# Yogesh352/llmsys-project-flashattn

Measured on AMD Instinct MI355X. Metric: FlashAttn fwd TFLOP/s (+ HBM GB/s) at (B,H,N,d)=(8,16,4096,64); 1/2/4/8 GPU, higher is better.
Workload: dtype bf16; 1 GPU; flash_attention_fwd c3; B=8, H=16, N=4096, d=64, causal=False, output=fp32 O, parallelism=bh-shard x1 (strong)

## Files before the change

### include/minitorch_hip.h

```cpp
#ifndef MINITORCH_HIP_H
#define MINITORCH_HIP_H

#include <stdint.h>
#include <stdbool.h>

#ifdef __cplusplus
extern "C" {
#endif

enum { MT_F32 = 0, MT_BF16 = 1, MT_BF16_F32OUT = 2 };

const char* mt_last_error(void);
int mt_abi_version(void);
int mt_flash_set_kernel_policy(int policy);
int mt_flash_get_kernel_policy(void);
int64_t mt_scratch_bytes(void);
int mt_scratch_release(void);

int mt_flash_attn_fwd(int dtype, int causal, const void* q, const void* k, const void* v,
                      void* o, float* m, float* l, int64_t B, int64_t H, int64_t N, int64_t d,
                      const int64_t* q_strides, const int64_t* k_strides,
                      const int64_t* v_strides, const int64_t* o_strides, void* stream);

int mt_flash_attn_fwd_varlen(int dtype, int causal, const void* q, const void* k, const void* v,
                             void* o, float* m, float* l, int64_t B, int64_t H, int64_t N,
                             int64_t d, const int64_t* q_strides, const int64_t* k_strides,
                             const int64_t* v_strides, const int64_t* o_strides,
                             const int* kv_len, void* stream);

int64_t mt_flash_attn_bwd_workspace_bytes(int64_t B, int64_t H, int64_t N, int64_t d);

int mt_flash_attn_bwd(int dtype, int causal, const void* q, const void* k, const void* v,
                      const void* o, const void* dout, const float* m, const float* l,
                      void* dq, void* dk, void* dv, int64_t B, int64_t H, int64_t N,
                      int64_t d, const int64_t* strides, void* workspace, void* stream);
int mt_flash_attn_bwd_varlen(int dtype, int causal, const void* q, const void* k, const void* v,
                             const void* o, const void* dout, const float* m, const float* l,
                             void* dq, void* dk, void* dv, int64_t B, int64_t H, int64_t N,
                             int64_t d, const int64_t* strides, const int* kv_len,
                             void* workspace, void* stream);
int mt_flash_attn_bwd_v3(int dtype, int causal, const void* q, const void* k, const void* v,
                         const void* o, const void* dout, const float* m, const float* l,
                         void* dq, void* dk, void* dv, int64_t B, int64_t H, int64_t N,
                         int64_t d, const int64_t* strides, const int* kv_len,
                         void* workspace, int64_t workspace_bytes, void* stream);

int mt_flash_attn_decode_splits(int dtype, int64_t B, int64_t H, int64_t Nq, int64_t Nk, int64_t d,
                                int64_t* span_keys, int64_t* tile_keys);
int64_t mt_flash_attn_decode_workspace_bytes(int dtype, int64_t B, int64_t H, int64_t Nq, int64_t Nk,
                                             int64_t d);
int mt_flash_attn_decode(int dtype, int causal, const void* q, const void* k_cache, const void* v_cache,
                         void* o, float* m, float* l, int64_t B, int64_t H, int64_t Nq, int64_t Nk,
                         int64_t d, const int64_t* q_strides, const int64_t* k_strides,
                         const int64_t* v_strides, const int64_t* o_strides, const int* kv_len,
                         void* workspace, int64_t workspace_bytes, void* stream);
int mt_flash_attn_decode_gqa_splits(int dtype, int64_t B, int64_t H, int64_t Hkv, int64_t Nq, int64_t Nk,
                                    int64_t d, int64_t* span_keys, int64_t* tile_keys);
int64_t mt_flash_attn_decode_gqa_workspace_bytes(int dtype, int64_t B, int64_t H, int64_t Hkv, int64_t Nq,
                                                 int64_t Nk, int64_t d);
int mt_flash_attn_decode_gqa(int dtype, int causal, const void* q, const void* k_cache, const void* v_cache,
                             void* o, float* m, float* l, int64_t B, int64_t H, int64_t Hkv, int64_t Nq,
                             int64_t Nk, int64_t d, const int64_t* q_strides, const int64_t* k_strides,
                             const int64_t* v_strides, const int64_t* o_strides, const int* kv_len,
                             void* workspace, int64_t workspace_bytes, void* stream);
int mt_flash_attn_extend_plan(int dtype, int64_t B, int64_t H, int64_t Hkv, int64_t Nq, int64_t Nk,
                              int64_t d, int64_t* block_queries, int64_t* tile_keys);
int mt_flash_attn_extend(int dtype, int causal, const void* q, const void* k_cache, const void* v_cache,
                         void* o, float* m, float* l, int64_t B, int64_t H, int64_t Hkv, int64_t Nq,
                         int64_t Nk, int64_t d, const int64_t* q_strides, const int64_t* k_strides,
                         const int64_t* v_strides, const int64_t* o_strides,
                         const int* kv_len, const int* q_len, void* stream);
int mt_kv_cache_append(int dtype, const void* k_new, const void* v_new, void* k_cache, void* v_cache,
                       int64_t B, int64_t H, int64_t Nq, int64_t Nmax, int64_t d,
                       const int64_t* knew_strides, const int64_t* vnew_strides,
                       const int64_t* kcache_strides, const int64_t* vcache_strides,
// ... 104 lines not shown
```

### llmsys-project-flashattn_amd/csrc/capi_flash.hip

```cpp
#include <stdarg.h>
#include <stdio.h>
#include <stdlib.h>
#include <string.h>

#include "../../include/minitorch_hip.h"
#include "fa_common.h"
#include <algorithm>
#include <atomic>
#include <mutex>
#include <vector>

namespace mt {
hipError_t launch_fwd_generic(const AttnArgs& a, bool bf16_io, bool vec, bool causal,
                              hipStream_t st, int ring);
hipError_t launch_fwd_fast(const AttnArgs& a, bool causal, int variant, hipStream_t st,
                           bool* handled);
hipError_t launch_fwd_v4(const AttnArgs& a, bool causal, int nw, bool pk, hipStream_t st,
                         bool* handled, int pair = 0);
hipError_t launch_fwd_v5(const AttnArgs& a, bool causal, int ahead, int var, hipStream_t st,
                         bool* handled);
hipError_t launch_fwd_v6(const AttnArgs& a, bool causal, int var, hipStream_t st, bool* handled);
hipError_t launch_fwd_d128(const AttnArgs& a, bool causal, int nw, bool dma, hipStream_t st,
                           bool* handled, int pair = 0);
hipError_t launch_fwd_d128v2(const AttnArgs& a, bool causal, int var, hipStream_t st, bool* handled);
hipError_t launch_bwd_bf16(const AttnArgs& a, bool causal, int variant, hipStream_t st, bool* handled);
hipError_t launch_bwd_generic(const AttnArgs& a, bool bf16_io, bool vec, bool causal,
                              hipStream_t st, int pair, bool ring, int64_t fused_slab);
int64_t bwd_fused_ws_bytes(int64_t B, int64_t H, int64_t N);
int64_t ring_fused_ws_bytes(int64_t B, int64_t H, int64_t N);
int64_t bwd_fused_abi2_bytes(int64_t B, int64_t H, int64_t N);
#ifdef MT_DIAGNOSTICS
hipError_t launch_fwd_v4_deep(const AttnArgs& a, bool causal, bool pk, hipStream_t st);
hipError_t launch_fwd_v4_ablation(const AttnArgs& a, int abl, hipStream_t st);
#endif

static thread_local char g_err[512] = "";

enum : int {
  kPolDefault = 0,
  kPolGeneric = 1,
  kPolFast8 = 2, kPolFast4 = 3, kPolFastSp8 = 4, kPolFastSp4 = 5, kPolFastPp = 6,
  kPolV4w4 = 21, kPolV4w8 = 22, kPolV4Pk8 = 23, kPolV4Pk4 = 24, kPolV4DeepPk = 25,
  kPolV4Deep = 26,
  kPolV4Pair4 = 50, kPolV4Pair8 = 51, kPolD128Pair4 = 52, kPolD128Pair8 = 53,
  kPolV4PairLF4 = 63, kPolV4PairLF8 = 64, kPolD128PairLF8 = 65,
  kPolV5a2 = 27, kPolV5a4 = 28, kPolV5a6 = 29, kPolV5NoUnroll = 31, kPolV5Dma = 35,
  kPolV5w8 = 36, kPolV5w8Dma = 37, kPolV5w4Reg = 38, kPolV5Prio = 39, kPolV5Scalar = 46,
  kPolV5Stagger = 47, kPolV5ScalarStagger = 48, kPolV5StaggerPrio = 49, kPolV5VKeep = 54,
  kPolV5VKeepPrio = 55, kPolV5Defer = 56, kPolV5Defer3 = 57, kPolV5Defer4 = 58,
  kPolV5AsmDma = 61,
  kPolV5Causal8 = 67, kPolV5Causal4 = 68,
  kPolD128w8 = 32, kPolD128w4 = 33, kPolD128Dma8 = 44, kPolD128Dma4 = 45,
  kPolBwdPipe = 40, kPolBwdQ32 = 43, kPolBwdQ64OneWave = 62,
  kPolBwdQ64Dma = 66, kPolBwdQ64Dma8 = 69,
  kPolBwdStagger = 70,
  kPolBwdDqPf = 71,
  kPolBwdMix0 = 74,
  kPolBwdMix4 = 75,
  kPolV5Split = 76,
  kPolBwdQ128 = 77,
  kPolV5RowSum = 78, kPolV5RowSumNoKeep = 79,
  kPolV6 = 100, kPolV6RowSum = 102, kPolV6RowSumNoKeep = 103,
  kPolV6RowSumEven = 104,
  kPolV6Split = 105,
  kPolV6Causal = 106,
  kPolBwdPair = 107, kPolBwdPair8 = 108,
  kPolFwdF32TwoBarrier = 109, kPolFwdF32Ring = 110, kPolFwdF32RingPair = 111,
  kPolBwdGenNoPair = 112, kPolBwdGenPair = 113,
  kPolBwdF32Lds = 114,
  kPolBwdFused = 120,
  kPolBwdSplit = 121,
  kPolD128v2 = 130, kPolD128v2Vs = 131, kPolD128v2Prio = 132, kPolD128v2w4 = 133, kPolD128v2w4Vs = 134,
  kPolD128v2Ah3 = 135, kPolD128v2Ah4 = 136,
  kPolD128v2Causal = 137,
// ... 266 lines not shown
    if (pol >= 80 && pol <= 86) {
      static const int kAbl[7] = {12, 28, 4, 68, 132, 260, 6};
      var = kAbl[pol - 80];
    }
    if (pol == 97) var = 2;
    if (pol == 98) var = v5::kDefault | 1048576;
    if (pol >= 91 && pol <= 96 && a.d == 64) {
      *handled = true;
      return launch_fwd_v4_ablation(a, pol - 90, st);
    }
#endif
    if (var >= 0) e = launch_fwd_v5(a, false, ahead, var, st, handled);
  }
  if (!*handled && pol == kPolDefault && causal && a.d == 64 &&
      (int64_t)((a.N + 511) / 512 + 1) / 2 * a.B * a.H >= 256)
  {
    const bool w4 = !a.o_f32 && (int64_t)((a.N + 255) / 256 + 1) / 2 * a.B * a.H >= 512;
    e = launch_fwd_v6(a, true, a.o_f32 ? 610 : w4 ? (98 | 16384) : 98, st, handled);
    if (!*handled) e = launch_fwd_v5(a, true, 2, v5::kDefault, st, handled);
  }
  if (!*handled && pol == kPolDefault && a.d == 64)
    e = launch_fwd_v4(a, causal, causal && N >= 8192 ? 8 : 4, !causal, st, handled,
                      causal ? 2 : 0);
  if (!*handled && a.d == 128) {
    int nw = -1, pair = 0;
    bool dma = false;
    if (pol == kPolDefault) e = launch_fwd_d128v2(a, causal, causal ? 32 : 0, st, handled);
    switch (*handled ? -1 : pol) {
      case kPolDefault: nw = 8; pair = causal ? 2 : 0; break;
      case kPolD128w8: nw = 8; break;
      case kPolD128w4: nw = 4; break;
      case kPolD128Dma8: nw = 8; dma = true; break;
      case kPolD128Dma4: nw = 4; dma = true; break;
      case kPolD128Pair4: nw = 4; pair = 1; break;
      case kPolD128Pair8: nw = 8; pair = 1; break;
      case kPolV4PairLF4: nw = 4; pair = 2; break;
      case kPolV4PairLF8: case kPolD128PairLF8: nw = 8; pair = 2; break;
      default: break;
    }
    if (nw > 0) e = launch_fwd_d128(a, causal, nw, dma, st, handled, pair);
  }
  if (!*handled) {
    int var = 2;
    if (pol >= kPolFast8 && pol <= kPolFastPp) var = pol;
#ifdef MT_DIAGNOSTICS
    if (pol >= 10 && pol <= 15) var = pol;
#endif
    e = launch_fwd_fast(a, causal, var, st, handled);
  }
  return e;
}
#endif

static hipError_t fwd_bf16_dispatch(const AttnArgs& a, bool causal, int pol, hipStream_t st,
                                    bool* handled) {
#ifdef MT_DIAGNOSTICS
  if (pol != kPolDefault && pol != kPolBwdFused && pol != kPolBwdSplit)
    return fwd_bf16_dispatch_ab(a, causal, pol, st, handled);
#endif
  (void)pol;
  *handled = false;
  hipError_t e = hipSuccess;
  const int N = a.N;
  const int64_t bh = (int64_t)a.B * a.H;
  if (a.d == 64) {
    if (!causal) {
      if (N % 64 == 0 && (int64_t)((N + 255) / 256) * bh >= 512)
        e = launch_fwd_v6(a, false, 66 | 16384, st, handled);
      else if ((int64_t)((N + 511) / 512) * bh >= 256)
        e = launch_fwd_v6(a, false, N % 64 ? 66 | 65536 : 66, st, handled);
      if (!*handled) e = launch_fwd_v6(a, false, 18, st, handled);
    } else {
      const int64_t w4grid = (int64_t)((N + 255) / 256 + 1) / 2 * bh;
      const int64_t w8grid = (int64_t)((N + 511) / 512 + 1) / 2 * bh;
      const int rg = N % 64 ? 65536 : 0;
      if (!a.o_f32 && w4grid >= 256) e = launch_fwd_v6(a, true, (98 | 16384) | rg, st, handled);
      else if (a.o_f32 && !rg && w8grid >= 256) e = launch_fwd_v6(a, true, 610, st, handled);
    }
    if (!*handled)
      e = launch_fwd_v4(a, causal, causal && N >= 8192 ? 8 : 4, !causal, st, handled, causal ? 2 : 0);
  }
  if (!*handled && a.d == 128) e = launch_fwd_d128v2(a, causal, causal ? 32 : 0, st, handled);
  if (!*handled && a.d == 128) e = launch_fwd_d128(a, causal, 8, false, st, handled, causal ? 2 : 0);
  if (!*handled) e = launch_fwd_fast(a, causal, 2, st, handled);
  return e;
}

}

using namespace mt;

extern "C" {

const char* mt_last_error(void) { return g_err; }
int mt_flash_set_kernel_policy(int policy) {
  if (!policy_valid(policy))
    return set_error("mt_flash_set_kernel_policy: unknown policy %d", policy);
  g_kernel_policy.store(policy, std::memory_order_relaxed);
  return 0;
}
int mt_flash_get_kernel_policy(void) { return g_kernel_policy.load(std::memory_order_relaxed); }
int mt_abi_version(void) { return 3; }

int mt_flash_attn_fwd(int dtype, int causal, const void* q, const void* k, const void* v,
                      void* o, float* m, float* l, int64_t B, int64_t H, int64_t N, int64_t d,
                      const int64_t* q_strides, const int64_t* k_strides,
                      const int64_t* v_strides, const int64_t* o_strides, void* stream) {
  return mt_flash_attn_fwd_varlen(dtype, causal, q, k, v, o, m, l, B, H, N, d, q_strides,
                                  k_strides, v_strides, o_strides, nullptr, stream);
}

int mt_flash_attn_fwd_varlen(int dtype, int causal, const void* q, const void* k, const void* v,
                             void* o, float* m, float* l, int64_t B, int64_t H, int64_t N,
                             int64_t d, const int64_t* q_strides, const int64_t* k_strides,
                             const int64_t* v_strides, const int64_t* o_strides,
                             const int* kv_len, void* stream) {
  const bool f32o = dtype == MT_BF16_F32OUT;
  if (f32o) dtype = MT_BF16;
  if (check_sizes(dtype, B, H, N, d)) return 1;
  if (!q || !k || !v || !o) return set_error("mt_flash_attn_fwd: null tensor pointer");
  AttnArgs a;
  memset(&a, 0, sizeof(a));
  a.q = q; a.k = k; a.v = v; a.out = o; a.m = m; a.l = l;
  a.kv_len = kv_len;
  a.o_f32 = f32o ? 1 : 0;
#ifdef MT_DIAGNOSTICS
  if (const char* kn = getenv("MT_KNOB")) a.knob = atoi(kn);
#endif
  fill_strides(a.sq, q_strides, H, N, d);
  fill_strides(a.sk, k_strides, H, N, d);
  fill_strides(a.sv, v_strides, H, N, d);
  fill_strides(a.so, o_strides, H, N, d);
  a.B = (int)B; a.H = (int)H; a.N = (int)N; a.d = (int)d;
  a.scale = (float)(1.0 / sqrt((double)d));
  a.scale_log2 = (float)(1.4426950408889634 / sqrt((double)d));
  const int es = dtype == MT_BF16 ? 2 : 4;
  const bool vec = vec_ok(d, es, {a.sq, a.sk, a.sv, a.so}, {q, k, v, o});
  if (f32o && !vec_ok(d, 4, {a.so}, {o}))
    return set_error("mt_flash_attn_fwd: an fp32 O needs 16-B aligned rows (d and O strides multiples of 4)");
  hipStream_t st = (hipStream_t)stream;
  const int pol = g_kernel_policy.load(std::memory_order_relaxed);
  if (dtype == MT_BF16 && vec && pol != kPolGeneric && !kv_len) {
    const int64_t dp = pad_dim(d);
    if (dp) {
      const int64_t oes = f32o ? 4 : 2;
      bool declined = false;
      const hipError_t e = for_head_groups(B, H, N * dp * (3 * 2 + oes), [&](int64_t b0, int64_t h0, int64_t nb, int64_t nh) -> hipError_t {
        if (declined) return hipSuccess;
        const int64_t nel = nb * nh * N * dp;
        char* buf = (char*)pad_scratch((size_t)(nel * (3 * 2 + oes)), st);
        if (!buf) { declined = true; return hipSuccess; }
        AttnArgs ap = a;
        ap.B = (int)nb; ap.H = (int)nh;
        ap.q = buf; ap.k = buf + nel * 2; ap.v = buf + nel * 4; ap.out = buf + nel * 6;
        int64_t* ps[4] = {ap.sq, ap.sk, ap.sv, ap.so};
// ... 303 lines not shown
```

### llmsys-project-flashattn_amd/csrc/fa_fwd_v6.hip

```cpp
#include "fa_fwd_bf16.h"

#ifndef V6ABL
#define V6ABL 0
#endif
#ifndef V6NT
#define V6NT 1
#endif

namespace mt {

namespace {

using namespace fwdbf16;
constexpr int D = 64;
constexpr int kBK = 64;
constexpr int TILE = kBK * D;
constexpr int kKSlots = 4, kVSlots = 2;
constexpr int kNW = 8;
constexpr int kBQ = 64 * kNW;
constexpr float kLimit = 1.8446744e19f;
constexpr float kThr = 8.0f;

typedef __attribute__((address_space(3))) s16x4 lds_s16x4;
typedef __attribute__((ext_vector_type(8))) short s16x8;
typedef __attribute__((ext_vector_type(4))) float f32x4;
typedef __attribute__((ext_vector_type(2))) float f32x2;
typedef __attribute__((ext_vector_type(8))) _Float16 f16x8;
typedef __attribute__((ext_vector_type(2))) _Float16 f16x2;
typedef __attribute__((ext_vector_type(4))) unsigned u32x4;

struct Blk6 {
  f32x4 s[4][2];
};
struct Pf6 {
  bf16x8 p[2];
};

__device__ __forceinline__ f32x4 mma16(const bf16x8& a, const bf16x8& b, const f32x4& c) {
  return __builtin_amdgcn_mfma_f32_16x16x32_bf16(a, b, c, 0, 0, 0);
}
template <bool H>
__device__ __forceinline__ f32x4 mma_pv(const bf16x8& a, const bf16x8& b, const f32x4& c) {
  if (!H) return mma16(a, b, c);
  return __builtin_amdgcn_mfma_f32_16x16x32_f16(__builtin_bit_cast(f16x8, a), __builtin_bit_cast(f16x8, b), c, 0, 0, 0);
}

__device__ __forceinline__ u32x4 vcvt_read(const bf16* tile, int tid) {
  return *(const u32x4*)((const char*)tile + tid * 16);
}
__device__ __forceinline__ void vcvt_write(bf16* tile, int tid, const u32x4& x) {
  u32x4 y;
#pragma unroll
  for (int j = 0; j < 4; ++j) {
    const f32x2 f = {__uint_as_float(x[j] << 16), __uint_as_float(x[j] & 0xffff0000u)};
    y[j] = __builtin_bit_cast(unsigned, __builtin_convertvector(f, f16x2));
  }
  *(u32x4*)((char*)tile + tid * 16) = y;
}

// ... 59 lines not shown

template <bool SOFT, bool PS, bool RS = false, bool EV = false, bool H = false, bool PK = false>
__device__ __forceinline__ void qk6(const bf16* sk, const int (&ko)[2], const bf16x8 (&qf)[2][2], Blk6& S,
                                    const f32x4 (&ci)[2], const Blk6& s_in, int kk, float c2,
                                    const float (&nmc)[2], f32x2 (&acc)[2], Pf6& pf) {
  bf16x8 kf[8];
  kf[0] = kread6(sk, ko, 0);
  kf[1] = kread6(sk, ko, 1);
  f32x2 ep, ec;
#pragma unroll
  for (int m = 0; m < 16; ++m) {
    const int f = m >> 1, kb = f >> 1, ks = f & 1, qh = m & 1;
    if (!(m & 1) && f + 2 < 8) kf[f + 2] = ((V6ABL & 1) && SOFT && f + 2 >= 4) ? kf[(f - 2) ^ 1] : kread6(sk, ko, f + 2);
    S.s[kb][qh] = mma16(kf[f], qf[qh][ks], ks ? S.s[kb][qh] : ci[qh]);
    if (SOFT) sm6_slot<PS, RS, EV, H, PK>(m, s_in, kk, c2, nmc, acc, pf, ep, ec);
    __builtin_amdgcn_sched_barrier(0);
  }
  if (SOFT && EV) sm6_fin<true, H>(ep, 7, acc, pf);
}

template <bool SOFT, int KEEP, bool PS, bool RS = false, bool EV = false, bool H = false, bool PK = false>
__device__ __forceinline__ void pv6(const bf16* sv, const int (&vo)[4], f32x4 (&O)[4][2], const Pf6& plo,
                                    const Pf6& phi, const Blk6& s_in, int kk, float c2,
                                    const float (&nmc)[2], f32x2 (&acc)[2], Pf6& pf, bf16x8 (&vk)[8],
                                    f32x4 (&R)[2]) {
  constexpr short one = H ? 0x3c00 : 0x3f80;
  const bf16x8 ones = __builtin_bit_cast(bf16x8, s16x8{one, one, one, one, one, one, one, one});
  bf16x8 vf_own[8];
  bf16x8(&vf)[8] = KEEP ? vk : vf_own;
  if (KEEP != 2) {
    vf[0] = vread6(sv, vo, 0);
    vf[1] = vread6(sv, vo, 1);
  }
  f32x2 ep, ec;
#pragma unroll
  for (int m = 0; m < 16; ++m) {
    const int f = m >> 1, hv = f >> 2, db = f & 3, qh = m & 1;
    if (KEEP != 2 && !(m & 1) && f + 2 < 8) vf[f + 2] = ((V6ABL & 8) && SOFT && f + 2 >= 4) ? vf[f - 2] : vread6(sv, vo, f + 2);
    O[db][qh] = mma_pv<H>(vf[f], (hv ? phi : plo).p[qh], O[db][qh]);
    if (RS && db == 0 && !((V6ABL & 2) && SOFT)) R[qh] = mma_pv<H>(ones, (hv ? phi : plo).p[qh], R[qh]);
    if (SOFT) sm6_slot<PS, RS, EV, H, PK>(m, s_in, kk, c2, nmc, acc, pf, ep, ec);
    __builtin_amdgcn_sched_barrier(0);
  }
  if (SOFT && EV) sm6_fin<true, H>(ep, 7, acc, pf);
}

__device__ __forceinline__ float quad_max(float x) {
  x = fmaxf(x, __shfl_xor(x, 16));
  return fmaxf(x, __shfl_xor(x, 32));
}
__device__ __forceinline__ float quad_sum(float x) {
  x += __shfl_xor(x, 16);
  return x + __shfl_xor(x, 32);
}
__device__ __forceinline__ float lane_max6(const Blk6& s, int qh) {
  float m = fmaxf(fmaxf(s.s[0][qh][0], s.s[0][qh][1]), s.s[0][qh][2]);
#pragma unroll
  for (int kb = 0; kb < 4; ++kb)
#pragma unroll
    for (int r = (kb ? 0 : 3); r < 4; ++r) m = fmaxf(m, s.s[kb][qh][r]);
  return m;
}

__device__ __forceinline__ void dma6(uint32_t lds, __amdgpu_buffer_rsrc_t rs, int go, int step) {
  unsigned keep;
  asm volatile(
      "s_mov_b32 %0, m0\n\ts_mov_b32 m0, %2\n\ts_nop 0\n\t"
      "buffer_load_dwordx4 %1, %3, 0 offen lds\n\ts_mov_b32 m0, %0"
      : "=&s"(keep)
      : "v"(go + step), "s"(lds), "s"(rs)
      : "memory");
}

__device__ __forceinline__ void dma6s(uint32_t lds, __amdgpu_buffer_rsrc_t rs, int go, int soff) {
  unsigned keep;
  asm volatile(
      "s_mov_b32 %0, m0\n\ts_mov_b32 m0, %2\n\ts_nop 0\n\t"
      "buffer_load_dwordx4 %1, %3, %4 offen lds\n\ts_mov_b32 m0, %0"
      : "=&s"(keep)
      : "v"(go), "s"(lds), "s"(rs), "s"(soff)
      : "memory");
}

}

template <int VAR>
__global__ __launch_bounds__(64 * kNW, 1) void fa_fwd_bf16_v6(AttnArgs p, int nqb) {
  constexpr bool PS = VAR & 1, RS = VAR & 2, EV = RS && (VAR & 8), SPLIT = VAR & 16, CAUSAL = VAR & 32;
  constexpr bool WIDE = VAR & 64;
  constexpr bool NOBAR = VAR & 128;
  constexpr bool DUAL = VAR & 256;
  constexpr bool H = VAR & 512;
  constexpr bool STAMP = VAR & 1024;
  constexpr bool ODMA = (VAR & 2048) && !SPLIT && !DUAL;
  constexpr int PFLIP = (VAR & 4096) ? 3 : (VAR & 8192) ? 2 : 0;
  constexpr bool W4 = (VAR & 16384) && !SPLIT && !DUAL;
  constexpr bool PK = (VAR & 32768) && !PS;
  constexpr bool RG = VAR & 65536;
  static_assert(!RG || (!SPLIT && !DUAL && !PS && (CAUSAL || !W4)), "ragged N: the 8-wave non-causal and the causal forms");
  constexpr bool RGM = RG && !CAUSAL;
  constexpr int NCV = W4 ? 2 : 1;
  static_assert(!(SPLIT && CAUSAL), "split keys: non-causal");
  static_assert(!DUAL || CAUSAL, "dual halves: causal");
  static_assert(!H || (CAUSAL && !DUAL && !PS && RS && !EV), "fp16 PV: the causal default form");
  constexpr int VS = H ? 4 : kVSlots;
  constexpr int K1 = (VAR & 4) ? 0 : 1, K2 = (VAR & 4) ? 0 : 2;
  constexpr int NWQ = (SPLIT || DUAL || W4) ? 4 : kNW;
  constexpr int LPT = ODMA ? 2 : kNW / NWQ;
  constexpr int BQ = 64 * NWQ;
  extern __shared__ __attribute__((aligned(16))) char smem_raw[];

  const int tid = threadIdx.x, lane = tid & 63;
  const int wave = __builtin_amdgcn_readfirstlane(tid >> 6);
  const int g = lane >> 4, i16 = lane & 15;
  const int N = p.N;
  const int half = (SPLIT || DUAL) ? (wave >> 2) : 0;
  const int wq = (SPLIT || DUAL) ? (wave & 3) : wave;
  const int Nk = SPLIT ? N / 2 : N;
  bf16* const sK = (bf16*)smem_raw + half * (kKSlots + VS) * TILE;
  bf16* const sV = sK + kKSlots * TILE;

  const int nblk = gridDim.x, hw = blockIdx.x;
  const int xcd = hw & 7, slot = hw >> 3, qd = nblk >> 3, rm = nblk & 7;
  const int logical = (xcd < rm ? xcd * (qd + 1) : rm * (qd + 1) + (xcd - rm) * qd) + slot;
  const int nunit = DUAL ? nqb / 4 : CAUSAL ? (nqb + 1) / 2 : nqb;
  const int bh = logical / nunit, qb = logical % nunit;
  const int b = bh / p.H, hh = bh % p.H;

  const bf16* Qg = (const bf16*)p.q + b * p.sq[0] + hh * p.sq[1];
  const bf16* Kg = (const bf16*)p.k + b * p.sk[0] + hh * p.sk[1] + (int64_t)(SPLIT ? half : 0) * Nk * p.sk[2];
  const bf16* Vg = (const bf16*)p.v + b * p.sv[0] + hh * p.sv[1] + (int64_t)(SPLIT ? half : 0) * Nk * p.sv[2];
  const int skn = (int)p.sk[2], svn = (int)p.sv[2];
  const __amdgpu_buffer_rsrc_t rk =
      __builtin_amdgcn_make_buffer_rsrc((void*)Kg, (short)0, ((Nk - 1) * skn + D) * 2, 0x00020000);
  const __amdgpu_buffer_rsrc_t rv =
      __builtin_amdgcn_make_buffer_rsrc((void*)Vg, (short)0, ((Nk - 1) * svn + D) * 2, 0x00020000);

  int ko[2], vo[4];
#pragma unroll
  for (int ks = 0; ks < 2; ++ks) ko[ks] = k_swz<D>(i16, 4 * ks + g);
  {
    const int q = i16 >> 2, pp = i16 & 3, row = 4 * g + q;
#pragma unroll
    for (int db = 0; db < 4; ++db)
      vo[db] = row * D + (((2 * db + (pp >> 1)) ^ (((row >> 1) & 3) << 1)) * 8) + 4 * (pp & 1);
  }
  auto prow = [&](int i) __attribute__((always_inline)) { return W4 ? 8 * (wq + 4 * i) : 8 * (LPT * wq + i); };
  constexpr int NDO = W4 ? 1 : LPT;
  int kdo[NDO], vdo[NDO];
#pragma unroll
  for (int i = 0; i < NDO; ++i) {
    const int dr = prow(i) + (lane >> 3), dc = lane & 7;
    kdo[i] = (dr * skn + (dc ^ ((dr >> 1) & 7)) * 8) * 2;
// ... 278 lines not shown
        const int qf0 = qw + 32 * blk;
        if (CAUSAL && (qf0 + 31 < t * kBK || qf0 >= N)) continue;
        Blk6 S;
        f32x2 acc[2] = {f32x2{0.f, 0.f}, f32x2{0.f, 0.f}};
        Pf6 plo, phi, dpf;
        const float z[2] = {0.f, 0.f};
        qk6<false, false>(sK, ko, blk ? qfB : qfA, S, ci0, S, 0, c2, z, acc, dpf);
        if (RGM && t * kBK + kBK > Nk) {
#pragma unroll
          for (int kb = 0; kb < 4; ++kb)
#pragma unroll
            for (int qh = 0; qh < 2; ++qh)
#pragma unroll
              for (int r = 0; r < 4; ++r)
                if (t * kBK + 16 * kb + 4 * g + r >= Nk) S.s[kb][qh][r] = -INFINITY;
        }
        if (CAUSAL && t * kBK + kBK - 1 > qf0) {
#pragma unroll
          for (int kb = 0; kb < 4; ++kb)
#pragma unroll
            for (int qh = 0; qh < 2; ++qh)
#pragma unroll
              for (int r = 0; r < 4; ++r)
                if (t * kBK + 16 * kb + 4 * g + r > qf0 + 16 * qh + i16) S.s[kb][qh][r] = -INFINITY;
        }
        float(&m)[2] = blk ? mB : mA;
        float(&l)[2] = blk ? pB : pA;
        f32x4(&O)[4][2] = blk ? OB : OA;
        float nmc[2];
#pragma unroll
        for (int qh = 0; qh < 2; ++qh) {
          const float tmax = quad_max(lane_max6(S, qh));
          if (__builtin_amdgcn_ballot_w64((tmax - m[qh]) * c2e > kThr)) {
            const float m_new = fmaxf(m[qh], tmax);
            const float alpha = m[qh] == -INFINITY ? 0.f : __builtin_amdgcn_exp2f((m[qh] - m_new) * c2e);
            m[qh] = m_new;
#pragma unroll
            for (int db = 0; db < 4; ++db) O[db][qh] *= alpha;
            l[qh] *= alpha;
          }
          nmc[qh] = -(m[qh] * c2e);
        }
#pragma unroll
        for (int i = 0; i < 8; ++i) sm6_fin(sm6_exp<false>(S, 0, i, c2e, nmc), i, acc, plo);
#pragma unroll
        for (int i = 0; i < 8; ++i) sm6_fin(sm6_exp<false>(S, 1, i, c2e, nmc), i, acc, phi);
#pragma unroll
        for (int qh = 0; qh < 2; ++qh) l[qh] += acc[qh][0] + acc[qh][1];
        f32x2 d2[2];
        f32x4 dR[2];
        pv6<false, 0, false>(sV, vo, O, plo, phi, S, 0, c2, nmc, d2, dpf, vk, dR);
      }
    }
  }
  if (SPLIT) {
    __syncthreads();
    float4* xch = (float4*)smem_raw + wq * 18 * 64 + lane;
    if (half) {
#pragma unroll
      for (int db = 0; db < 4; ++db)
#pragma unroll
        for (int qh = 0; qh < 2; ++qh) {
          const f32x4 a = OA[db][qh], o = OB[db][qh];
          xch[(2 * db + qh) * 64] = make_float4(a[0], a[1], a[2], a[3]);
          xch[(8 + 2 * db + qh) * 64] = make_float4(o[0], o[1], o[2], o[3]);
        }
      xch[16 * 64] = make_float4(mA[0], mA[1], mB[0], mB[1]);
      xch[17 * 64] = make_float4(pA[0], pA[1], pB[0], pB[1]);
    }
    __syncthreads();
    if (half) return false;
    const float4 tm = xch[16 * 64], tp = xch[17 * 64];
    const float om[4] = {tm.x, tm.y, tm.z, tm.w}, op[4] = {tp.x, tp.y, tp.z, tp.w};
#pragma unroll
    for (int blk = 0; blk < 2; ++blk)
#pragma unroll
      for (int qh = 0; qh < 2; ++qh) {
        float& m = blk ? mB[qh] : mA[qh];
        float& l = blk ? pB[qh] : pA[qh];
        const float n = fmaxf(m, om[2 * blk + qh]);
        const float a0 = __builtin_amdgcn_exp2f((m - n) * c2e), a1 = __builtin_amdgcn_exp2f((om[2 * blk + qh] - n) * c2e);
#pragma unroll
        for (int db = 0; db < 4; ++db) {
          const float4 u = xch[((blk ? 8 : 0) + 2 * db + qh) * 64];
          f32x4& o = (blk ? OB : OA)[db][qh];
          o = o * a0 + f32x4{u.x, u.y, u.z, u.w} * a1;
        }
        l = l * a0 + op[2 * blk + qh] * a1;
        m = n;
      }
  }

#pragma unroll
  for (int blk = 0; blk < 2; ++blk) {
#pragma unroll
    for (int qh = 0; qh < 2; ++qh) {
      const int q = qw + 32 * blk + 16 * qh + i16;
      const float l = quad_sum(blk ? pB[qh] : pA[qh]);
      const float m = blk ? mB[qh] : mA[qh];
      const float inv = 1.f / l;
      const f32x4(&O)[4][2] = blk ? OB : OA;
      if (V6ABL & 16) {
        float t = 0.f;
#pragma unroll
        for (int db = 0; db < 4; ++db) t += O[db][qh][0] * inv + O[db][qh][1] + O[db][qh][2] + O[db][qh][3];
        if (t == 1.2345e-30f) p.l[0] = t;
        if (q < N && g == 0) {
          const int64_t row = (int64_t)bh * N + q;
          if (p.m) p.m[row] = m * p.scale;
          if (p.l) p.l[row] = l;
        }
        continue;
      }
      if (WIDE && !p.o_f32) {
        bf16* Ob = (bf16*)p.out + b * p.so[0] + hh * p.so[1] + (int64_t)min(q, N - 1) * p.so[2];
        typedef __attribute__((ext_vector_type(4))) __bf16 bf16x4;
#pragma unroll
        for (int k = 0; k < 2; ++k) {
          const f32x4 &x = O[2 * k][qh], &y = O[2 * k + 1][qh];
          const uint2 ux = __builtin_bit_cast(uint2, bf16x4{(bf16)(x[0] * inv), (bf16)(x[1] * inv), (bf16)(x[2] * inv), (bf16)(x[3] * inv)});
          const uint2 uy = __builtin_bit_cast(uint2, bf16x4{(bf16)(y[0] * inv), (bf16)(y[1] * inv), (bf16)(y[2] * inv), (bf16)(y[3] * inv)});
          const auto rx = __builtin_amdgcn_permlane16_swap(ux.x, uy.x, false, false);
          const auto ry = __builtin_amdgcn_permlane16_swap(ux.y, uy.y, false, false);
          if (q < N) {
            u32x4* dst = (u32x4*)(Ob + 32 * k + 16 * (g & 1) + 4 * (g & 2));
            const u32x4 val = {rx[0], ry[0], rx[1], ry[1]};
            if (V6NT) __builtin_nontemporal_store(val, dst);
            else *dst = val;
          }
        }
      }
      if (q < N) {
        const ORow Og = o_row(p, b, hh, q);
        if (V6NT && p.o_f32) {
#pragma unroll
          for (int db = 0; db < 4; ++db)
            __builtin_nontemporal_store(f32x4{O[db][qh][0] * inv, O[db][qh][1] * inv, O[db][qh][2] * inv,
                                              O[db][qh][3] * inv}, (f32x4*)((float*)Og.p + 16 * db + 4 * g));
        } else if (!WIDE || p.o_f32) {
#pragma unroll
          for (int db = 0; db < 4; ++db)
            store4(Og, 16 * db + 4 * g, O[db][qh][0] * inv, O[db][qh][1] * inv, O[db][qh][2] * inv,
                   O[db][qh][3] * inv);
        }
        if (g == 0) {
          const int64_t row = (int64_t)bh * N + q;
          if (p.m) p.m[row] = m * (PS ? p.scale / c2 : p.scale);
          if (p.l) p.l[row] = l;
        }
      }
    }
  }
  return bad;
  };

  if (DUAL) {
    const int light = 2 * qb + half, heavy = nqb - 1 - light;
    bool bad = run_block(light * BQ, 1);
    __syncthreads();
    bad = run_block(heavy * BQ, 1) || bad;
    if (__syncthreads_or(bad)) {
      run_block(light * BQ, 2);
      __syncthreads();
      run_block(heavy * BQ, 2);
    }
  } else if (CAUSAL) {
    const int heavy = nqb - 1 - qb;
    run_block(qb * BQ, 0);
    if (heavy != qb) {
      __syncthreads();
      run_block(heavy * BQ, 0);
    }
  } else {
    run_block(qb * BQ, 0);
  }
}

hipError_t launch_fwd_v6(const AttnArgs& a, bool causal, int var, hipStream_t st, bool* handled) {
  *handled = false;
  const bool one_wg = (var & (1 << 20)) != 0;
  var &= ~(1 << 20);
  const bool split = (var & 16) != 0;
  const bool dual = (var & 256) != 0;
  const bool rg = (var & 65536) != 0;
  if (causal != ((var & 32) != 0) || a.d != 64 || (!rg && a.N % kBK != 0) || a.N < 2 * kBK) return hipSuccess;
  if (split && (a.N % (2 * kBK) != 0 || a.N < 4 * kBK)) return hipSuccess;
  if (dual && a.N % (4 * kBQ / 2) != 0) return hipSuccess;
  const int64_t lim = (int64_t)1 << 31;
  if (((int64_t)a.N + 2 * kBK) * a.sk[2] * 2 >= lim || ((int64_t)a.N + 2 * kBK) * a.sv[2] * 2 >= lim)
    return hipSuccess;
  *handled = true;
  const size_t smem = (size_t)(split || dual ? 2 : 1) * (kKSlots + (var & 512 ? 4 : kVSlots)) * TILE * sizeof(bf16);
  void (*kern)(AttnArgs, int) = nullptr;
  switch (var) {
    case 66: kern = fa_fwd_bf16_v6<66>; break;
    case 18: kern = fa_fwd_bf16_v6<18>; break;
    case 98: kern = fa_fwd_bf16_v6<98>; break;
    case 610: kern = fa_fwd_bf16_v6<610>; break;
    case 16482: kern = fa_fwd_bf16_v6<16482>; break;
    case 16450: kern = fa_fwd_bf16_v6<16450>; break;
    case 65602: kern = fa_fwd_bf16_v6<65602>; break;
    case 65634: kern = fa_fwd_bf16_v6<65634>; break;
    case 82018: kern = fa_fwd_bf16_v6<82018>; break;
#ifdef MT_DIAGNOSTICS
    case 354: kern = fa_fwd_bf16_v6<354>; break;
    case 1090: kern = fa_fwd_bf16_v6<1090>; break;
    case 2114: kern = fa_fwd_bf16_v6<2114>; break;
    case 3138: kern = fa_fwd_bf16_v6<3138>; break;
    case 4162: kern = fa_fwd_bf16_v6<4162>; break;
    case 8258: kern = fa_fwd_bf16_v6<8258>; break;
    case 5186: kern = fa_fwd_bf16_v6<5186>; break;
    case 32834: kern = fa_fwd_bf16_v6<32834>; break;
    case 102: kern = fa_fwd_bf16_v6<102>; break;
    case 16994: kern = fa_fwd_bf16_v6<16994>; break;
    case 16486: kern = fa_fwd_bf16_v6<16486>; break;
    case 16998: kern = fa_fwd_bf16_v6<16998>; break;
    case 614: kern = fa_fwd_bf16_v6<614>; break;
    case 194: kern = fa_fwd_bf16_v6<194>; break;
    case 2: kern = fa_fwd_bf16_v6<2>; break;
    case 34: kern = fa_fwd_bf16_v6<34>; break;
    case 82: kern = fa_fwd_bf16_v6<82>; break;
    case 0: kern = fa_fwd_bf16_v6<0>; break;
    case 6: kern = fa_fwd_bf16_v6<6>; break;
    case 10: kern = fa_fwd_bf16_v6<10>; break;
    case 1: kern = fa_fwd_bf16_v6<1>; break;
#endif
    default: return hipErrorInvalidValue;
  }
  const size_t smem_launch = one_wg && smem < 96 * 1024 ? (size_t)96 * 1024 : smem;
  hipError_t e = hipFuncSetAttribute((const void*)kern, hipFuncAttributeMaxDynamicSharedMemorySize, (int)smem_launch);
  if (e != hipSuccess) return e;
  const bool w4 = (var & 16384) != 0;
  const int bq = split || dual || w4 ? kBQ / 2 : kBQ;
  const int nqb = (a.N + bq - 1) / bq;
  const int64_t nblk = (int64_t)(dual ? nqb / 4 : causal ? (nqb + 1) / 2 : nqb) * a.B * a.H;
  if (nblk > 0x7fffffff) return hipErrorInvalidValue;
  hipLaunchKernelGGL(kern, dim3((unsigned)nblk), dim3(w4 ? 32 * kNW : 64 * kNW), smem_launch, st, a, nqb);
  return hipGetLastError();
}

}
```

### llmsys-project-flashattn_amd/minitorch/_hip.py

```python
from __future__ import annotations

import ctypes
import os
from typing import Optional, Sequence

_HERE = os.path.dirname(os.path.abspath(__file__))
LIB_PATH = os.environ.get("MT_HIP_LIB") or os.path.join(_HERE, "_lib", "libminitorch_hip.so")

MT_F32 = 0
MT_BF16 = 1

_lib = None

_i64 = ctypes.c_int64
_int = ctypes.c_int
_vp = ctypes.c_void_p
_fp = ctypes.POINTER(ctypes.c_float)
_i64p = ctypes.POINTER(ctypes.c_int64)
_ip = ctypes.POINTER(ctypes.c_int)
_vpp = ctypes.POINTER(ctypes.c_void_p)

_PROTOS = {
    "mt_last_error": (ctypes.c_char_p, []),
    "mt_abi_version": (_int, []),
    "mt_flash_set_kernel_policy": (_int, [_int]),
    "mt_flash_get_kernel_policy": (_int, []),
    "mt_scratch_bytes": (_i64, []),
    "mt_scratch_release": (_int, []),
    "mt_flash_attn_fwd": (_int, [_int, _int, _vp, _vp, _vp, _vp, _vp, _vp, _i64, _i64, _i64, _i64,
                                 _i64p, _i64p, _i64p, _i64p, _vp]),
    "mt_flash_attn_fwd_varlen": (_int, [_int, _int, _vp, _vp, _vp, _vp, _vp, _vp, _i64, _i64, _i64,
                                        _i64, _i64p, _i64p, _i64p, _i64p, _vp, _vp]),
    "mt_flash_attn_bwd_workspace_bytes": (_i64, [_i64, _i64, _i64, _i64]),
    "mt_flash_attn_bwd": (_int, [_int, _int, _vp, _vp, _vp, _vp, _vp, _vp, _vp, _vp, _vp, _vp,
                                 _i64, _i64, _i64, _i64, _i64p, _vp, _vp]),
    "mt_flash_attn_bwd_varlen": (_int, [_int, _int, _vp, _vp, _vp, _vp, _vp, _vp, _vp, _vp, _vp, _vp,
                                        _i64, _i64, _i64, _i64, _i64p, _vp, _vp, _vp]),
    "mt_flash_attn_bwd_v3": (_int, [_int, _int, _vp, _vp, _vp, _vp, _vp, _vp, _vp, _vp, _vp, _vp,
                                    _i64, _i64, _i64, _i64, _i64p, _vp, _vp, _i64, _vp]),
    "mt_flash_attn_decode_splits": (_int, [_int, _i64, _i64, _i64, _i64, _i64, _i64p, _i64p]),
    "mt_flash_attn_decode_workspace_bytes": (_i64, [_int, _i64, _i64, _i64, _i64, _i64]),
    "mt_flash_attn_decode": (_int, [_int, _int, _vp, _vp, _vp, _vp, _vp, _vp, _i64, _i64, _i64, _i64, _i64,
                                    _i64p, _i64p, _i64p, _i64p, _vp, _vp, _i64, _vp]),
    "mt_flash_attn_decode_gqa_splits": (_int, [_int, _i64, _i64, _i64, _i64, _i64, _i64, _i64p, _i64p]),
    "mt_flash_attn_decode_gqa_workspace_bytes": (_i64, [_int, _i64, _i64, _i64, _i64, _i64, _i64]),
    "mt_flash_attn_decode_gqa": (_int, [_int, _int, _vp, _vp, _vp, _vp, _vp, _vp, _i64, _i64, _i64, _i64, _i64, _i64,
                                        _i64p, _i64p, _i64p, _i64p, _vp, _vp, _i64, _vp]),
    "mt_flash_attn_extend_plan": (_int, [_int, _i64, _i64, _i64, _i64, _i64, _i64, _i64p, _i64p]),
    "mt_flash_attn_extend": (_int, [_int, _int, _vp, _vp, _vp, _vp, _vp, _vp, _i64, _i64, _i64, _i64, _i64, _i64,
                                    _i64p, _i64p, _i64p, _i64p, _vp, _vp, _vp]),
    "mt_kv_cache_append": (_int, [_int, _vp, _vp, _vp, _vp, _i64, _i64, _i64, _i64, _i64,
                                  _i64p, _i64p, _i64p, _i64p, _vp, _vp]),
    "mt_select_token": (_int, [_vp, _i64, _i64, _i64, ctypes.c_float, _i64, ctypes.c_uint64, _vp, _i64,
                               _vp, _vp, _vp, _vp, _i64, _vp, _vp]),
    "mt_attn_softmax_fw": (_int, [_vp, _vp, _vp, _i64, _i64, _i64, _i64, _i64p, _int, _vp]),
    "mt_attn_softmax_bw": (_int, [_vp, _vp, _vp, _i64, _i64, _vp]),
    "mt_layernorm_fw": (_int, [_vp, _vp, _vp, _vp, _vp, _vp, _i64, _i64, _vp]),
    "mt_bias_gelu_fw": (_int, [_vp, _vp, _vp, _i64, _i64, _vp]),
    "mt_bias_gelu_bw": (_int, [_vp, _vp, _vp, _vp, _i64, _i64, _vp]),
    "mt_dropout": (_int, [_vp, _vp, _i64, ctypes.c_float, ctypes.c_float, ctypes.c_uint64, _vp]),
    "mt_dropout_dseed": (_int, [_vp, _vp, _i64, ctypes.c_float, ctypes.c_float, _vp, _vp]),
    "mt_embedding_fw": (_int, [_vp, _vp, _vp, _i64, _i64, _i64, _vp]),
    "mt_embedding_bw": (_int, [_vp, _vp, _vp, _i64, _i64, _i64, _vp]),
    "mt_softmax_xent_fw": (_int, [_vp, _vp, _vp, _vp, _i64, _i64, _vp]),
    "mt_softmax_xent_bw": (_int, [_vp, _vp, _vp, _vp, _vp, _i64, _i64, _vp]),
    "mt_layernorm_bw_workspace_bytes": (_i64, [_i64, _i64]),
    "mt_layernorm_bw": (_int, [_vp] * 9 + [_i64, _i64, _vp, _vp]),
    "mt_tensor_map": (_int, [_int, _vp, _i64p, _i64p, _int, _vp, _i64p, _i64p, _int, _vp]),
    "mt_tensor_zip": (_int, [_int, _vp, _i64p, _i64p, _int, _vp, _i64p, _i64p, _int,
                             _vp, _i64p, _i64p, _int, _vp]),
    "mt_tensor_reduce": (_int, [_int, _vp, _i64p, _i64p, _vp, _i64p, _i64p, _int, _int,
                                ctypes.c_float, _vp]),
    "mt_matmul_f32": (_int, [_vp, _vp, _vp, _i64, _i64, _i64, _i64, _i64p, _i64p, _i64p, _vp]),
    "mt_rand_uniform": (_int, [_vp, _i64, ctypes.c_uint64, _vp]),
    "mt_adam_step": (_int, [_int, _vpp, _vpp, _vpp, _vpp, _i64p, ctypes.c_double, ctypes.c_double,
                            ctypes.c_double, ctypes.c_double, _vp]),
    "mt_adam_step_dstep": (_int, [_int, _vpp, _vpp, _vpp, _vpp, _i64p, ctypes.c_double, ctypes.c_double,
                                  ctypes.c_double, _vp, _vp]),
    "mt_set_gemm_backend": (None, [_int]),
    "mt_matmul_f32_plan": (_int, [_int, _i64, _i64, _i64, _i64, _i64p, _i64p, _i64p, _vp, _vp, _vp,
                                  ctypes.POINTER(ctypes.c_int32)]),
    "launch_attn_softmax": (None, [_fp, _fp, _int, _int, _int, _int, ctypes.c_bool, _vp]),
    "launch_attn_softmax_bw": (None, [_fp, _fp, _int, _int, _vp]),
# ... 121 lines not shown
def _check_dev(*ts) -> None:
    for t in ts:
        if not t.is_cuda:
            raise ValueError("HIP flash attention needs device (cuda) tensors")


def _kv_arg(kv_len, B, device):
    if kv_len is None:
        return None
    torch = _torch()
    kv = torch.as_tensor(kv_len, device=device).to(torch.int32).contiguous()
    if kv.shape != (B,):
        raise ValueError(f"kv_len must have shape ({B},), got {tuple(kv.shape)}")
    return kv


def flash_fwd(q, k, v, causal: bool = False, out=None, m=None, l=None, stream: Optional[int] = None,
              kv_len=None, out_dtype=None):
    torch = _torch()
    _check_dev(q, k, v)
    B, H, N, d = q.shape
    if k.shape != q.shape or v.shape != q.shape:
        raise ValueError(f"q/k/v shapes differ: {tuple(q.shape)} {tuple(k.shape)} {tuple(v.shape)}")
    if not (q.dtype == k.dtype == v.dtype):
        raise TypeError("q/k/v dtypes differ")
    code = dtype_code(q)
    f32o = q.dtype == torch.bfloat16 and (out_dtype == torch.float32 or
                                          (out is not None and out.dtype == torch.float32))
    if out is None:
        out = torch.empty_like(q, dtype=torch.float32 if f32o else q.dtype,
                               memory_format=torch.contiguous_format)
    if f32o:
        code = 2
    if m is None:
        m = torch.empty((B, H, N), dtype=torch.float32, device=q.device)
    if l is None:
        l = torch.empty((B, H, N), dtype=torch.float32, device=q.device)
    st = stream_ptr(q.device) if stream is None else stream
    kv = _kv_arg(kv_len, B, q.device)
    if kv is None:
        check(lib().mt_flash_attn_fwd(code, int(causal), q.data_ptr(), k.data_ptr(),
                                      v.data_ptr(), out.data_ptr(), m.data_ptr(), l.data_ptr(),
                                      B, H, N, d, strides3(q), strides3(k), strides3(v),
                                      strides3(out), st), "mt_flash_attn_fwd")
    else:
        check(lib().mt_flash_attn_fwd_varlen(code, int(causal), q.data_ptr(), k.data_ptr(),
                                             v.data_ptr(), out.data_ptr(), m.data_ptr(), l.data_ptr(),
                                             B, H, N, d, strides3(q), strides3(k), strides3(v),
                                             strides3(out), kv.data_ptr(), st),
              "mt_flash_attn_fwd_varlen")
    return out, m, l


def flash_bwd(q, k, v, o, do, m, l, causal: bool = False, dq=None, dk=None, dv=None,
              workspace=None, stream: Optional[int] = None, kv_len=None):
    torch = _torch()
    _check_dev(q, k, v, o, do, m, l)
    B, H, N, d = q.shape
    dq = torch.empty_like(q, memory_format=torch.contiguous_format) if dq is None else dq
    dk = torch.empty_like(k, memory_format=torch.contiguous_format) if dk is None else dk
    dv = torch.empty_like(v, memory_format=torch.contiguous_format) if dv is None else dv
    if workspace is None:
        nbytes = lib().mt_flash_attn_bwd_workspace_bytes(B, H, N, d)
        workspace = torch.empty(nbytes // 4, dtype=torch.float32, device=q.device)
    m = m.contiguous().float()
    l = l.contiguous().float()
    strides = (ctypes.c_int64 * 24)()
    for i, t in enumerate((q, k, v, o, do, dq, dk, dv)):
        s = strides3(t)
        strides[3 * i:3 * i + 3] = list(s)
    st = stream_ptr(q.device) if stream is None else stream
    kv = _kv_arg(kv_len, B, q.device)
    args = (dtype_code(q), int(causal), q.data_ptr(), k.data_ptr(), v.data_ptr(), o.data_ptr(),
            do.data_ptr(), m.data_ptr(), l.data_ptr(), dq.data_ptr(), dk.data_ptr(), dv.data_ptr(),
            B, H, N, d, strides)
    check(lib().mt_flash_attn_bwd_v3(*args, None if kv is None else kv.data_ptr(),
                                     workspace.data_ptr(), workspace.numel() * workspace.element_size(),
                                     st), "mt_flash_attn_bwd_v3")
    return dq, dk, dv


def _decode_code(q, out, out_dtype) -> int:
    torch = _torch()
    code = dtype_code(q)
    if q.dtype == torch.bfloat16 and (out_dtype == torch.float32 or
                                      (out is not None and out.dtype == torch.float32)):
        code = 2
    return code


def decode_splits(dtype: int, B: int, H: int, Nq: int, Nk: int, d: int, Hkv: Optional[int] = None):
    span, tile = ctypes.c_int64(0), ctypes.c_int64(0)
    n = lib().mt_flash_attn_decode_gqa_splits(dtype, B, H, H if Hkv is None else Hkv, Nq, Nk, d,
                                              ctypes.byref(span), ctypes.byref(tile))
    if n <= 0:
        raise ValueError(lib().mt_last_error().decode(errors="replace"))
    return n, span.value, tile.value


def decode_workspace_bytes(dtype: int, B: int, H: int, Nq: int, Nk: int, d: int, Hkv: Optional[int] = None) -> int:
    n = lib().mt_flash_attn_decode_gqa_workspace_bytes(dtype, B, H, H if Hkv is None else Hkv, Nq, Nk, d)
    if n < 0:
        raise ValueError(lib().mt_last_error().decode(errors="replace"))
    return int(n)


# ... 173 lines not shown
```

Before: 1178 TFLOP/s.

## Stage v6 forward output through LDS for row-contiguous coalesced stores

Adds an epilogue to the v6 forward kernel that normalizes the accumulators, transposes them through a per-wave shared-memory staging area with XOR swizzling, and writes each output row as contiguous 16-byte nontemporal stores, for both fp32 and bf16 output. It also computes m/l per row in the same epilogue. The aim is to replace the scattered MFMA-layout global writes of the fp32 O tensor with fully coalesced row writes. The cost is extra LDS traffic, wave barriers, and an added __syncthreads at the end of the main loop. Separately, the dispatch logic is refactored into a helper and a plan query API is exposed.

```diff
diff --git a/include/minitorch_hip.h b/include/minitorch_hip.h
--- a/include/minitorch_hip.h
+++ b/include/minitorch_hip.h
@@ -21,6 +21,8 @@
                       void* o, float* m, float* l, int64_t B, int64_t H, int64_t N, int64_t d,
                       const int64_t* q_strides, const int64_t* k_strides,
                       const int64_t* v_strides, const int64_t* o_strides, void* stream);
+
+int mt_flash_attn_fwd_plan(int dtype, int causal, int64_t B, int64_t H, int64_t N, int64_t d);
 
 int mt_flash_attn_fwd_varlen(int dtype, int causal, const void* q, const void* k, const void* v,
                              void* o, float* m, float* l, int64_t B, int64_t H, int64_t N,
diff --git a/llmsys-project-flashattn_amd/csrc/capi_flash.hip b/llmsys-project-flashattn_amd/csrc/capi_flash.hip
--- a/llmsys-project-flashattn_amd/csrc/capi_flash.hip
+++ b/llmsys-project-flashattn_amd/csrc/capi_flash.hip
@@ -20,6 +20,7 @@
 hipError_t launch_fwd_v5(const AttnArgs& a, bool causal, int ahead, int var, hipStream_t st,
                          bool* handled);
 hipError_t launch_fwd_v6(const AttnArgs& a, bool causal, int var, hipStream_t st, bool* handled);
+bool fwd_v6_takes(const AttnArgs& a, bool causal, int var);
 hipError_t launch_fwd_d128(const AttnArgs& a, bool causal, int nw, bool dma, hipStream_t st,
                            bool* handled, int pair = 0);
 hipError_t launch_fwd_d128v2(const AttnArgs& a, bool causal, int var, hipStream_t st, bool* handled);
@@ -392,6 +393,23 @@
 }
 #endif
 
+static void fwd_v6_default_vars(const AttnArgs& a, bool causal, int (&vars)[2]) {
+  const int N = a.N;
+  const int64_t bh = (int64_t)a.B * a.H;
+  vars[0] = vars[1] = 0;
+  if (!causal) {
+    if (N % 64 == 0 && (int64_t)((N + 255) / 256) * bh >= 512) vars[0] = 66 | 16384;
+    else if ((int64_t)((N + 511) / 512) * bh >= 256) vars[0] = N % 64 ? 66 | 65536 : 66;
+    vars[1] = 18;
+  } else {
+    const int64_t w4grid = (int64_t)((N + 255) / 256 + 1) / 2 * bh;
+    const int64_t w8grid = (int64_t)((N + 511) / 512 + 1) / 2 * bh;
+    const int rg = N % 64 ? 65536 : 0;
+    if (!a.o_f32 && w4grid >= 256) vars[0] = (98 | 16384) | rg;
+    else if (a.o_f32 && !rg && w8grid >= 256) vars[0] = 610;
+  }
+}
+
 static hipError_t fwd_bf16_dispatch(const AttnArgs& a, bool causal, int pol, hipStream_t st,
                                     bool* handled) {
 #ifdef MT_DIAGNOSTICS
@@ -402,20 +420,16 @@
   *handled = false;
   hipError_t e = hipSuccess;
   const int N = a.N;
-  const int64_t bh = (int64_t)a.B * a.H;
   if (a.d == 64) {
     if (!causal) {
-      if (N % 64 == 0 && (int64_t)((N + 255) / 256) * bh >= 512)
-        e = launch_fwd_v6(a, false, 66 | 16384, st, handled);
-      else if ((int64_t)((N + 511) / 512) * bh >= 256)
-        e = launch_fwd_v6(a, false, N % 64 ? 66 | 65536 : 66, st, handled);
-      if (!*handled) e = launch_fwd_v6(a, false, 18, st, handled);
+      int vars[2];
+      fwd_v6_default_vars(a, false, vars);
+      for (int i = 0; i < 2 && !*handled; ++i)
+        if (vars[i]) e = launch_fwd_v6(a, false, vars[i], st, handled);
     } else {
-      const int64_t w4grid = (int64_t)((N + 255) / 256 + 1) / 2 * bh;
-      const int64_t w8grid = (int64_t)((N + 511) / 512 + 1) / 2 * bh;
-      const int rg = N % 64 ? 65536 : 0;
-      if (!a.o_f32 && w4grid >= 256) e = launch_fwd_v6(a, true, (98 | 16384) | rg, st, handled);
-      else if (a.o_f32 && !rg && w8grid >= 256) e = launch_fwd_v6(a, true, 610, st, handled);
+      int vars[2];
+      fwd_v6_default_vars(a, true, vars);
+      if (vars[0]) e = launch_fwd_v6(a, true, vars[0], st, handled);
     }
     if (!*handled)
       e = launch_fwd_v4(a, causal, causal && N >= 8192 ? 8 : 4, !causal, st, handled, causal ? 2 : 0);
@@ -441,6 +455,25 @@
 }
 int mt_flash_get_kernel_policy(void) { return g_kernel_policy.load(std::memory_order_relaxed); }
 int mt_abi_version(void) { return 3; }
+
+int mt_flash_attn_fwd_plan(int dtype, int causal, int64_t B, int64_t H, int64_t N, int64_t d) {
+  const bool f32o = dtype == MT_BF16_F32OUT;
+  if (check_sizes(f32o ? MT_BF16 : dtype, B, H, N, d)) return -1;
+  if ((dtype != MT_BF16 && !f32o) || d != 64) return 0;
+  AttnArgs a;
+  memset(&a, 0, sizeof(a));
+  a.o_f32 = f32o ? 1 : 0;
+  fill_strides(a.sq, nullptr, H, N, d);
+  fill_strides(a.sk, nullptr, H, N, d);
+  fill_strides(a.sv, nullptr, H, N, d);
+  fill_strides(a.so, nullptr, H, N, d);
+  a.B = (int)B; a.H = (int)H; a.N = (int)N; a.d = (int)d;
+  int vars[2];
+  fwd_v6_default_vars(a, causal != 0, vars);
+  for (int i = 0; i < 2; ++i)
+    if (vars[i] && fwd_v6_takes(a, causal != 0, vars[i])) return vars[i];
+  return 0;
+}
 
 int mt_flash_attn_fwd(int dtype, int causal, const void* q, const void* k, const void* v,
                       void* o, float* m, float* l, int64_t B, int64_t H, int64_t N, int64_t d,
diff --git a/llmsys-project-flashattn_amd/csrc/fa_fwd_v6.hip b/llmsys-project-flashattn_amd/csrc/fa_fwd_v6.hip
--- a/llmsys-project-flashattn_amd/csrc/fa_fwd_v6.hip
+++ b/llmsys-project-flashattn_amd/csrc/fa_fwd_v6.hip
@@ -1,3 +1,5 @@
+#include <type_traits>
+
 #include "fa_fwd_bf16.h"
 
 #ifndef V6ABL
@@ -5,6 +7,9 @@
 #endif
 #ifndef V6NT
 #define V6NT 1
+#endif
+#ifndef V6ROWS
+#define V6ROWS 3
 #endif
 
 namespace mt {
@@ -170,6 +175,11 @@
 __device__ __forceinline__ float quad_sum(float x) {
   x += __shfl_xor(x, 16);
   return x + __shfl_xor(x, 32);
+}
+__device__ __forceinline__ void wave_sync() {
+  __builtin_amdgcn_fence(__ATOMIC_RELEASE, "wavefront");
+  __builtin_amdgcn_wave_barrier();
+  __builtin_amdgcn_fence(__ATOMIC_ACQUIRE, "wavefront");
 }
 __device__ __forceinline__ float lane_max6(const Blk6& s, int qh) {
   float m = fmaxf(fmaxf(s.s[0][qh][0], s.s[0][qh][1]), s.s[0][qh][2]);
@@ -217,6 +227,8 @@
   constexpr bool RG = VAR & 65536;
   static_assert(!RG || (!SPLIT && !DUAL && !PS && (CAUSAL || !W4)), "ragged N: the 8-wave non-causal and the causal forms");
   constexpr bool RGM = RG && !CAUSAL;
+  constexpr bool ROWS32 = (V6ROWS & 1) && !DUAL && !(V6ABL & 16);
+  constexpr bool ROWS16 = (V6ROWS & 2) && !DUAL && !(V6ABL & 16);
   constexpr int NCV = W4 ? 2 : 1;
   static_assert(!(SPLIT && CAUSAL), "split keys: non-causal");
   static_assert(!DUAL || CAUSAL, "dual halves: causal");
@@ -601,6 +613,7 @@
         pv6<false, 0, false>(sV, vo, O, plo, phi, S, 0, c2, nmc, d2, dpf, vk, dR);
       }
     }
+    if ((ROWS32 || ROWS16) && !SPLIT) __syncthreads();
   }
   if (SPLIT) {
     __syncthreads();
@@ -640,6 +653,85 @@
       }
   }
 
+  if (p.o_f32 ? ROWS32 : ROWS16) {
+    char* const stg = smem_raw + (SPLIT ? 72 * 1024 + wq * 4096 : wave * 4096);
+    float lq[2][2];
+#pragma unroll
+    for (int qh = 0; qh < 2; ++qh) {
+      lq[0][qh] = quad_sum(pA[qh]);
+      lq[1][qh] = quad_sum(pB[qh]);
+    }
+    {
+      const float mm = (g & 2) ? ((g & 1) ? mB[1] : mB[0]) : ((g & 1) ? mA[1] : mA[0]);
+      const float ll = (g & 2) ? ((g & 1) ? lq[1][1] : lq[1][0]) : ((g & 1) ? lq[0][1] : lq[0][0]);
+      const int q = qw + lane;
+      if (q < N) {
+        const int64_t row = (int64_t)bh * N + q;
+        if (p.m) p.m[row] = mm * (PS ? p.scale / c2 : p.scale);
+        if (p.l) p.l[row] = ll;
+      }
+    }
+    auto rows = [&](auto f32_c, auto full_c) __attribute__((always_inline)) {
+      constexpr bool F32 = decltype(f32_c)::value, FULL = decltype(full_c)::value;
+      constexpr int ES = F32 ? 4 : 2;
+      constexpr int RPI = F32 ? 4 : 8;
+      constexpr int NK = 16 / RPI;
+      constexpr int RB = 64 * ES;
+      const int rl = F32 ? g : lane >> 3, cl = F32 ? i16 : lane & 7;
+      u32x4 val[4][NK];
+#pragma unroll
+      for (int blk = 0; blk < 2; ++blk) {
+#pragma unroll
+        for (int qh = 0; qh < 2; ++qh) {
+          const float inv = 1.f / lq[blk][qh];
+          const f32x4(&O)[4][2] = blk ? OB : OA;
+          wave_sync();
+#pragma unroll
+          for (int db = 0; db < 4; ++db) {
+            const f32x4 x = O[db][qh] * inv;
+            if (F32) {
+              *(f32x4*)(stg + i16 * RB + (((4 * db + g) ^ i16) << 4)) = x;
+            } else {
+              typedef __attribute__((ext_vector_type(4))) __bf16 bf16x4;
+              *(uint2*)(stg + i16 * RB + (((2 * db + (g >> 1)) ^ (i16 >> 1)) << 4) + 8 * (g & 1)) =
+                  __builtin_bit_cast(uint2, bf16x4{(bf16)x[0], (bf16)x[1], (bf16)x[2], (bf16)x[3]});
+            }
+          }
+          wave_sync();
+#pragma unroll
+          for (int k = 0; k < NK; ++k) {
+            const int r = rl + RPI * k;
+            val[2 * blk + qh][k] = *(const u32x4*)(stg + r * RB + ((cl ^ (F32 ? r : r >> 1)) << 4));
+          }
+        }
+      }
+      wave_sync();
+      const int64_t ors = p.so[2] * ES;
+      char* const ob = (char*)p.out + (b * p.so[0] + hh * p.so[1] + (int64_t)(qw + rl) * p.so[2]) * ES + 16 * cl;
+#pragma unroll
+      for (int gk = 0; gk < 4 * NK; ++gk) {
+        const int r0 = 16 * (gk / NK) + RPI * (gk % NK);
+        if (FULL || qw + r0 + rl < N) {
+          u32x4* dst = (u32x4*)(ob + r0 * ors);
+          if (V6NT) __builtin_nontemporal_store(val[gk / NK][gk % NK], dst);
+          else *dst = val[gk / NK][gk % NK];
+        }
+      }
+    };
+    const bool full = qw + 64 <= N;
+    if (p.o_f32) {
+      if (ROWS32) {
+        if (full) rows(std::true_type{}, std::true_type{});
+        else rows(std::true_type{}, std::false_type{});
+      }
+    } else {
+      if (ROWS16) {
+        if (full) rows(std::false_type{}, std::true_type{});
+        else rows(std::false_type{}, std::false_type{});
+      }
+    }
+    return bad;
+  }
 #pragma unroll
   for (int blk = 0; blk < 2; ++blk) {
 #pragma unroll
@@ -725,19 +817,25 @@
   }
 }
 
+bool fwd_v6_takes(const AttnArgs& a, bool causal, int var) {
+  var &= ~(1 << 20);
+  const bool split = (var & 16) != 0;
+  const bool dual = (var & 256) != 0;
+  const bool rg = (var & 65536) != 0;
+  if (causal != ((var & 32) != 0) || a.d != 64 || (!rg && a.N % kBK != 0) || a.N < 2 * kBK) return false;
+  if (split && (a.N % (2 * kBK) != 0 || a.N < 4 * kBK)) return false;
+  if (dual && a.N % (4 * kBQ / 2) != 0) return false;
+  const int64_t lim = (int64_t)1 << 31;
+  return ((int64_t)a.N + 2 * kBK) * a.sk[2] * 2 < lim && ((int64_t)a.N + 2 * kBK) * a.sv[2] * 2 < lim;
+}
+
 hipError_t launch_fwd_v6(const AttnArgs& a, bool causal, int var, hipStream_t st, bool* handled) {
   *handled = false;
   const bool one_wg = (var & (1 << 20)) != 0;
   var &= ~(1 << 20);
   const bool split = (var & 16) != 0;
   const bool dual = (var & 256) != 0;
-  const bool rg = (var & 65536) != 0;
-  if (causal != ((var & 32) != 0) || a.d != 64 || (!rg && a.N % kBK != 0) || a.N < 2 * kBK) return hipSuccess;
-  if (split && (a.N % (2 * kBK) != 0 || a.N < 4 * kBK)) return hipSuccess;
-  if (dual && a.N % (4 * kBQ / 2) != 0) return hipSuccess;
-  const int64_t lim = (int64_t)1 << 31;
-  if (((int64_t)a.N + 2 * kBK) * a.sk[2] * 2 >= lim || ((int64_t)a.N + 2 * kBK) * a.sv[2] * 2 >= lim)
-    return hipSuccess;
+  if (!fwd_v6_takes(a, causal, var)) return hipSuccess;
   *handled = true;
   const size_t smem = (size_t)(split || dual ? 2 : 1) * (kKSlots + (var & 512 ? 4 : kVSlots)) * TILE * sizeof(bf16);
   void (*kern)(AttnArgs, int) = nullptr;
diff --git a/llmsys-project-flashattn_amd/minitorch/_hip.py b/llmsys-project-flashattn_amd/minitorch/_hip.py
--- a/llmsys-project-flashattn_amd/minitorch/_hip.py
+++ b/llmsys-project-flashattn_amd/minitorch/_hip.py
@@ -29,6 +29,7 @@
     "mt_scratch_release": (_int, []),
     "mt_flash_attn_fwd": (_int, [_int, _int, _vp, _vp, _vp, _vp, _vp, _vp, _i64, _i64, _i64, _i64,
                                  _i64p, _i64p, _i64p, _i64p, _vp]),
+    "mt_flash_attn_fwd_plan": (_int, [_int, _int, _i64, _i64, _i64, _i64]),
     "mt_flash_attn_fwd_varlen": (_int, [_int, _int, _vp, _vp, _vp, _vp, _vp, _vp, _i64, _i64, _i64,
                                         _i64, _i64p, _i64p, _i64p, _i64p, _vp, _vp]),
     "mt_flash_attn_bwd_workspace_bytes": (_i64, [_i64, _i64, _i64, _i64]),
@@ -256,6 +257,13 @@
     return out, m, l
 
 
+def fwd_plan(dtype: int, causal: bool, B: int, H: int, N: int, d: int) -> int:
+    kid = lib().mt_flash_attn_fwd_plan(dtype, int(causal), B, H, N, d)
+    if kid < 0:
+        check(1, "mt_flash_attn_fwd_plan")
+    return kid
+
+
 def flash_bwd(q, k, v, o, do, m, l, causal: bool = False, dq=None, dk=None, dv=None,
               workspace=None, stream: Optional[int] = None, kv_len=None):
     torch = _torch()
```

After: 1179 TFLOP/s, median of 6. About the same (+0.1%).
